# Youncy-Hu/MAGE

Measured on AMD Instinct MI355X. Metric: generated frames/sec (64x64, 16-frame clips), higher is better.
Workload: dtype bf16

## Files before the change

### mage_amd/config.py

```python
from __future__ import annotations

import contextlib
import dataclasses
import os
from typing import Iterator

__all__ = ["Config", "ENV", "get", "override", "lib_option", "lib_options", "lib_flag", "LIB_OPTIONS"]


@dataclasses.dataclass(frozen=True)
class Config:
    qk_fuse: bool = True
    mlp_fuse: bool = True
    ln_fold: bool = True
    stream_16bit: bool = True
    attn_split: bool = True
    frame_table: bool = True
    auto_graph: bool = True
    encode_split: bool = True
    decode_table: bool = True
    decode_split: bool = True
    decode_taps8: bool = True
    decode_resblock_fusion: bool = True
    decode_head_fusion: bool = True
    decode_phase_merge: bool = True
    decode_relu_fold: bool = True
    train_f32_branch: bool = False
    train_wgrad_transpose: bool = False
    train_emit: bool = True
    train_dual: bool = True
    train_taps: bool = True
    train_enc_split: bool = True


ENV = {
    "ln_fold": ("MAGE_NO_LN_FOLD", False),
    "qk_fuse": ("MAGE_NO_QK_FUSE", False),
    "mlp_fuse": ("MAGE_NO_MLP_FUSE", False),
    "stream_16bit": ("MAGE_STREAM_FP32", False),
    "attn_split": ("MAGE_ATTN_SPLIT_FP32", False),
    "frame_table": ("MAGE_NO_FRAME_TABLE", False),
    "auto_graph": ("MAGE_NO_AUTO_GRAPH", False),
    "encode_split": ("MAGE_ENCODE_FP32", False),
    "decode_table": ("MAGE_NO_DECODE_TABLE", False),
    "decode_split": ("MAGE_DECODE_FP32", False),
    "decode_taps8": ("MAGE_DECODE_NO_TAPS8", False),
    "decode_resblock_fusion": ("MAGE_DECODE_NO_RESBLOCK_FUSION", False),
    "decode_head_fusion": ("MAGE_DECODE_NO_HEAD_FUSION", False),
    "decode_phase_merge": ("MAGE_DECODE_NO_PHASE_MERGE", False),
    "decode_relu_fold": ("MAGE_DECODE_NO_RELU_FOLD", False),
    "train_f32_branch": ("MAGE_TRAIN_F32_BRANCH", True),
    "train_wgrad_transpose": ("MAGE_WGRAD_TRANSPOSE", True),
    "train_emit": ("MAGE_TRAIN_NO_EMIT", False),
    "train_dual": ("MAGE_TRAIN_NO_DUAL", False),
    "train_taps": ("MAGE_TRAIN_NO_TAPS", False),
    "train_enc_split": ("MAGE_TRAIN_ENC_FP32", False),
}

LIB_OPTIONS = ("gemm_no_4w", "gemm_no_4h", "gemm_4h_plain", "gemm4_train_forms", "gemm_no_8phase", "gemm_no_taps8", "gemm_no_narrow", "gemm_no_narrow_few", "gemm_no_small",
               "gemm_small_m", "gemm_stagger_groups", "gemm_stagger_percent", "gemm_stagger_forced",
               "gemm4_stagger_groups", "gemm4_stagger_percent", "attn_no_mfma", "attn_no_fewq", "vq_no_mfma", "conv_no_tile")


def _set(v) -> bool:
    return bool(v) and v != "0"


def _from_env() -> Config:
    kw = {}
    for field, (var, when_set) in ENV.items():
# ... 75 lines not shown
```

### mage_amd/csrc/gemm4.hip

```cpp
#include <cstdio>
#include <cstdlib>
#include <utility>

#include "gemm_shared.h"
#include "gemm4_regs.h"
#include "attn_mfma.h"

namespace {

struct Gemm4Args {
    const void* A;
    const void* W;
    void* Y;
    const float* bias;
    const float* ln_stats;
    const float* ln_colsum;
    const void* residual;
    float* ln_part;
    void* y2;
    int M, N, K, lda, ldw, ldy, ldr, ldy2, y_dtype, a_off, y_off;
    int ntiles_n, ntiles;
    int stagger_groups, stagger_sleeps;
    alignas(16) int attn_axis;
    float attn_scale;
// ... 23 lines not shown
#ifdef MAGE4_MFMA32
template <int B, bool ZERO, bool CLOB>
__device__ __forceinline__ void g4_mfma32(const u32x4& w, const u32x4& x) {
    if constexpr (ZERO && CLOB) asm volatile("v_mfma_f32_32x32x16_bf16 a[%c2:%c3], %0, %1, 0" ::"v"(w), "v"(x), "i"(16 * B), "i"(16 * B + 15) : G4_ALL_ACC);
    else if constexpr (ZERO) asm volatile("v_mfma_f32_32x32x16_bf16 a[%c2:%c3], %0, %1, 0" ::"v"(w), "v"(x), "i"(16 * B), "i"(16 * B + 15));
    else if constexpr (CLOB) asm volatile("v_mfma_f32_32x32x16_bf16 a[%c2:%c3], %0, %1, a[%c2:%c3]" ::"v"(w), "v"(x), "i"(16 * B), "i"(16 * B + 15) : G4_ALL_ACC);
    else asm volatile("v_mfma_f32_32x32x16_bf16 a[%c2:%c3], %0, %1, a[%c2:%c3]" ::"v"(w), "v"(x), "i"(16 * B), "i"(16 * B + 15));
}
#endif
typedef unsigned g4_u32x2 __attribute__((ext_vector_type(2)));
template <bool HF>
__device__ __forceinline__ f32x4 g4_epi_qk(const u32x4& k, const u32x4& q) {
    f32x4 d;
    if constexpr (HF) asm volatile("s_nop 1\n\tv_mfma_f32_16x16x32_f16 %0, %1, %2, 0\n\ts_nop 15" : "=&v"(d) : "v"(k), "v"(q));
    else asm volatile("s_nop 1\n\tv_mfma_f32_16x16x32_bf16 %0, %1, %2, 0\n\ts_nop 15" : "=&v"(d) : "v"(k), "v"(q));
    return d;
}
#define G4_EPI_PV(OP)                                                                                                                               \
    asm volatile("s_nop 1\n\t" OP " %0, %2, %4, 0\n\t" OP " %1, %3, %4, 0\n\t" OP " %0, %2, %5, %0\n\t" OP " %1, %3, %5, %1\n\ts_nop 15"           \
                 : "=&v"(o0), "=&v"(o1)                                                                                                             \
                 : "v"(__builtin_bit_cast(g4_u32x2, vt0)), "v"(__builtin_bit_cast(g4_u32x2, vt1)), "v"(__builtin_bit_cast(g4_u32x2, phi)),          \
                   "v"(__builtin_bit_cast(g4_u32x2, plo)))
template <bool HF>
__device__ __forceinline__ void g4_epi_pv(const ashort4& vt0, const ashort4& vt1, const ashort4& phi, const ashort4& plo, f32x4& o0, f32x4& o1) {
    if constexpr (HF) G4_EPI_PV("v_mfma_f32_16x16x16_f16");
    else G4_EPI_PV("v_mfma_f32_16x16x16_bf16");
}

template <bool SWAP, int I, bool ZERO, bool CLOB, bool HF>
__device__ __forceinline__ void g4_mm(const u32x4& w, const u32x4& x) {
    if constexpr (SWAP) g4_mfma<I, ZERO, CLOB, HF>(x, w);
    else g4_mfma<I, ZERO, CLOB, HF>(w, x);
}
template <int ACT, int EK, int LN, bool RB, bool HF, bool QF>
__device__ __forceinline__ void gemm4_body(const Gemm4Args& g) {
    static_assert(EK != EK_GENERAL, "lean epilogue kinds");
    static_assert(!QF || (LN == LN_CONSUME && ACT == MAGE_ACT_NONE), "fused attention: the LayerNorm-consuming in_proj");
    static_assert(!HF || (LN != LN_DUAL && LN != LN_GELUBWD), "f16 form: the generation path's epilogues");
    typedef std::conditional_t<HF, f16_t, unsigned short> H16;
    extern __shared__ __attribute__((aligned(16))) char smem[];
    g4_claim_accumulators();
    const int tid = threadIdx.x;
    const int lane = tid & 63;
    const int wave = __builtin_amdgcn_readfirstlane(tid >> 6);
    const int nwg8 = gridDim.x >> 3;
    const int xcd = blockIdx.x & 7, li = blockIdx.x >> 3;
    const int q8 = g.ntiles >> 3, r8 = g.ntiles & 7;
    const int chunk0 = xcd < r8 ? xcd * (q8 + 1) : r8 * (q8 + 1) + (xcd - r8) * q8;
    const int chunk1 = chunk0 + q8 + (xcd < r8 ? 1 : 0);
    const int nk = g.K >> 6;
    int c_tile = chunk0 + li;
    if (c_tile >= chunk1) return;
    const int last_tile = c_tile + ((chunk1 - 1 - c_tile) / nwg8) * nwg8;

    const int lr = lane >> 3, lp = lane & 7;
    unsigned voffA[8], voffW[8];
    [[maybe_unused]] auto frame_row = [&](int R) { return g.attn_axis == 1 ? ((R & 15) << 4) + (R >> 4) : R; };
#pragma unroll
    for (int u = 0; u < 8; ++u) {
        const int r = u * 8 + lr;
        const int ch = lp ^ ((r >> 1) & 7);
        voffA[u] = (unsigned)((QF ? frame_row(wave * 64 + r) : r) * g.lda * 2 + ch * 16 + 8192 - u * 1024);
        voffW[u] = (unsigned)(r * g.ldw * 2 + ch * 16 + 8192 - u * 1024);
    }
    auto a_base = [&](int tile) { return (const char*)g.A + ((long)((tile / g.ntiles_n) * 256 + (QF ? 0 : wave * 64)) + g.a_off) * g.lda * 2 - 4096; };
    auto w_base = [&](int tile) { return (const char*)g.W + (long)((tile % g.ntiles_n) * (QF ? 384 : 256) + wave * 64) * g.ldw * 2 - 4096; };
    [[maybe_unused]] auto w_base_v = [&](int tile) { return (const char*)g.W + (long)((tile % g.ntiles_n) * 384 + 256 + wave * 32) * g.ldw * 2 - 4096; };
    const char* a_src = a_base(c_tile);
    const char* w_src = w_base(c_tile);
    const char* a_next = a_src;
    const char* w_next = w_src;
    const unsigned lds0 = (unsigned)(uintptr_t)(__attribute__((address_space(3))) char*)smem + wave * 8192 + 4096;
    auto dma_m0 = [&](unsigned lds_group) __attribute__((always_inline)) {
        asm volatile("s_mov_b32 m0, %0\n\ts_nop 0" ::"s"(lds0 + lds_group) : "memory");
    };
    auto dma_m0w = [&](unsigned stage_off, bool half) __attribute__((always_inline)) { dma_m0(stage_off + G4_WOFF - (half ? wave * 4096 : 0)); };

    const int wm = wave >> 1, wn = wave & 1;
    const int l15 = lane & 15, grp = lane >> 4;
    const int rsw = (l15 >> 1) & 7;
    const int pc[2] = {((grp + 0) ^ rsw) * 16, ((grp + 4) ^ rsw) * 16};
    const int x_off = (wm * 128 + l15) * 128;
    const int w_off = G4_WOFF + (wn * 128 + l15) * 128;
    [[maybe_unused]] const int w_off_v = G4_WOFF + (wn * 64 + l15) * 128;
    u32x4 wf[2][8], xf[2][4];
    auto rd_w1 = [&](int buf, int stage, int t, int nt) __attribute__((always_inline)) {
        wf[buf][nt] = *(const u32x4*)(smem + stage * G4_STAGE + w_off + nt * 2048 + pc[t]);
    };
    [[maybe_unused]] auto rd_wv = [&](int buf, int stage, int t, int nt) __attribute__((always_inline)) {
        wf[buf][nt] = *(const u32x4*)(smem + stage * G4_STAGE + w_off_v + nt * 2048 + pc[t]);
    };
    auto rd_x1 = [&](int buf, int stage, int t, int mt) __attribute__((always_inline)) {
        xf[buf][mt & 3] = *(const u32x4*)(smem + stage * G4_STAGE + x_off + mt * 2048 + pc[t]);
    };

#ifdef MAGE4_MFMA32
    const int l31 = lane & 31, hi5 = lane >> 5;
    const int rsw32 = (l31 >> 1) & 7;
// ... 9 lines not shown
    if (g.stagger_groups > 1) {
        for (int w = (li % g.stagger_groups) * g.stagger_sleeps; w > 0; --w) __builtin_amdgcn_s_sleep(16);
    }
    dma_m0(0);
    g4_for<8>([&](auto u_) { g4_dma<decltype(u_)::value>(voffA[decltype(u_)::value], a_src); });
    dma_m0(G4_WOFF);
    g4_for<8>([&](auto u_) { g4_dma<decltype(u_)::value>(voffW[decltype(u_)::value], w_src); });
    a_src += 128;
    w_src += 128;
    dma_m0(G4_STAGE);
    g4_for<8>([&](auto u_) { g4_dma<decltype(u_)::value>(voffA[decltype(u_)::value], a_src); });
    dma_m0(G4_STAGE + G4_WOFF);
    g4_for<8>([&](auto u_) { g4_dma<decltype(u_)::value>(voffW[decltype(u_)::value], w_src); });
    a_src += 128;
    w_src += 128;
    __builtin_amdgcn_s_waitcnt(0x0F70);
    ring_barrier();
#ifdef MAGE4_MFMA32
#pragma unroll
    for (int b = 0; b < 4; ++b) { rd_w32(0, 0, 0, b); rd_x32(0, 0, 0, b); }
#else
#pragma unroll
    for (int nt = 0; nt < 8; ++nt) rd_w1(0, 0, 0, nt);
#pragma unroll
    for (int m = 0; m < 4; ++m) rd_x1(0, 0, 0, m);
#endif

    [[maybe_unused]] int it = 0;
    for (; c_tile < chunk1; c_tile += nwg8, ++it) {
        G4_STAMP(it, 0);
        const int tm = c_tile / g.ntiles_n, tn = c_tile - tm * g.ntiles_n;
        MAGE_DASSERT(c_tile >= 0 && c_tile < g.ntiles && tm * 256 < g.M && tn * (QF ? 384 : 256) < g.N);
        [[maybe_unused]] float ln_mean[8], ln_rstd[8];
        auto tile = [&](auto PH_) __attribute__((always_inline)) {
            constexpr int PH = decltype(PH_)::value;
            constexpr bool HALF = PH == 2, KEEP = PH == 1;
            constexpr int NW = HALF ? 4 : 8;
            const int m0 = ((MAGE4_ABL & 32) ? (int)blockIdx.x : tm) * 256 + wm * 128;
            const int n0 = QF ? tn * 384 + (HALF ? 256 + wn * 64 : wn * 128) : ((MAGE4_ABL & 32) ? 0 : tn) * 256 + wn * 128;
            [[maybe_unused]] const int ny0 = HALF ? tn * 128 + wn * 64 : n0;
            if constexpr (KEEP) {
                a_next = a_base(c_tile);
                w_next = w_base_v(c_tile);
            } else {
                const int nt_tile = c_tile + nwg8 > last_tile ? last_tile : c_tile + nwg8;
                a_next = a_base(nt_tile);
                w_next = w_base(nt_tile);
            }
            auto rd_w = [&](int buf, int stage, int t, int nt) __attribute__((always_inline)) {
                if constexpr (HALF) rd_wv(buf, stage, t, nt);
                else rd_w1(buf, stage, t, nt);
            };
            f32x4 biasm[2][4];
            [[maybe_unused]] f32x4 lns[2][4];
            [[maybe_unused]] f32x4 pl[4][2];
            [[maybe_unused]] int ql15 = l15, qgrp = grp;
            if constexpr (QF) asm volatile("" : "+v"(ql15), "+v"(qgrp));
            auto slab = [&](auto S_, auto FIRST_, auto LAST_, int j) __attribute__((always_inline)) {
                constexpr int S = decltype(S_)::value;
                constexpr bool FIRST = decltype(FIRST_)::value, LAST = decltype(LAST_)::value;
                constexpr int ACC0 = HALF ? 32 : 0;
                constexpr bool WH_ = LAST ? KEEP : HALF;
                constexpr int WU = WH_ ? 4 : 8;
                g4_for<4 * NW>([&](auto i_) {
                    constexpr int i = decltype(i_)::value, m = i / NW, nt = i % NW;
                    g4_mm<PH == 2, ACC0 + ((nt >> 2) * 8 + m) * 4 + (nt & 3), FIRST, i == 0, HF>(wf[0][nt], xf[0][m]);
                    __builtin_amdgcn_sched_barrier(0);
                    if constexpr (!(MAGE4_ABL & 4) && i < 4) {
                        rd_x1(1, S, 0, 4 + i);
                        __builtin_amdgcn_sched_barrier(0);
                    }
                    if constexpr (!(MAGE4_ABL & 2) && !FIRST && i == 4) {
                        dma_m0w((S ^ 1) * G4_STAGE, WH_);
                        __builtin_amdgcn_sched_barrier(0);
                    }
// ... 9 lines not shown
                        }
                    }
                });
                if constexpr (!(MAGE4_ABL & 2) && !FIRST && !HALF && WU == 8) {
                    g4_dma<7>(voffW[7], w_src);
                    __builtin_amdgcn_sched_barrier(0);
                }
                if constexpr (!(MAGE4_ABL & 8) && !FIRST) w_src = (j == nk - 2) ? w_next : w_src + 128;
                g4_for<4 * NW>([&](auto i_) {
                    constexpr int i = decltype(i_)::value, m = i / NW, nt = i % NW;
                    g4_mm<PH == 2, ACC0 + ((nt >> 2) * 8 + 4 + m) * 4 + (nt & 3), FIRST, i == 0, HF>(wf[0][nt], xf[1][m]);
                    __builtin_amdgcn_sched_barrier(0);
                    if constexpr (!(MAGE4_ABL & 4) && i < 4 + NW) {
                        if constexpr (i < 4) rd_x1(0, S, 1, i);
                        else rd_w(1, S, 1, i - 4);
                        __builtin_amdgcn_sched_barrier(0);
                    }
                });
                if constexpr (LAST) {
#pragma unroll
                    for (int b = 0; b < 4; ++b) {
                        if constexpr (PH == 2) {
                            biasm[0][0][b] = g.bias[n0 + b * 16 + l15];
                            lns[0][0][b] = g.ln_colsum[n0 + b * 16 + l15];
                            continue;
                        }
                        const int n = n0 + b * 16 + grp * 4;
                        biasm[0][b] = *(const f32x4*)(g.bias + n);
                        if constexpr (LN == LN_CONSUME) lns[0][b] = *(const f32x4*)(g.ln_colsum + n);
                    }
                    if constexpr (LN == LN_CONSUME && !HALF) {
#pragma unroll
                        for (int a = 0; a < 8; ++a) {
                            const long row = QF ? (long)tm * 256 + frame_row(wm * 128 + a * 16 + ql15) : (long)(m0 + a * 16 + l15);
                            const float2 st = *(const float2*)(g.ln_stats + 2 * row);
                            ln_mean[a] = st.x;
                            ln_rstd[a] = st.y;
                        }
                    }
                    __builtin_amdgcn_sched_barrier(0);
                }
                g4_for<4 * NW>([&](auto i_) {
                    constexpr int i = decltype(i_)::value, m = i / NW, nt = i % NW;
                    g4_mm<PH == 2, ACC0 + ((nt >> 2) * 8 + m) * 4 + (nt & 3), false, i == 0, HF>(wf[1][nt], xf[0][m]);
                    __builtin_amdgcn_sched_barrier(0);
                    if constexpr (!(MAGE4_ABL & 4) && i < 4) {
                        rd_x1(1, S, 1, 4 + i);
                        __builtin_amdgcn_sched_barrier(0);
                    }
                });
                if constexpr (MAGE4_ABL & 16) __builtin_amdgcn_s_waitcnt(0xC07F);
                else if constexpr (FIRST && QF) __builtin_amdgcn_s_waitcnt(PH == 1 ? 0x007C : 0x0070);
                else if constexpr (FIRST) __builtin_amdgcn_s_waitcnt(LN == LN_CONSUME ? 0x8074 : 0x8070);
                else __builtin_amdgcn_s_waitcnt(0x0070);
                ring_barrier();
                __builtin_amdgcn_sched_barrier(0);
                g4_for<4 * NW>([&](auto i_) {
                    constexpr int i = decltype(i_)::value, m = i / NW, nt = i % NW;
                    g4_mm<PH == 2, ACC0 + ((nt >> 2) * 8 + 4 + m) * 4 + (nt & 3), false, i == 0, HF>(wf[1][nt], xf[1][m]);
                    __builtin_amdgcn_sched_barrier(0);
                    if constexpr (!(MAGE4_ABL & 4) && i < 4 + NW && !LAST) {
                        if constexpr (i < 4) rd_x1(0, S ^ 1, 0, i);
                        else rd_w(0, S ^ 1, 0, i - 4);
                        __builtin_amdgcn_sched_barrier(0);
                    }
                    if constexpr (!(MAGE4_ABL & 2) && !LAST && !HALF) {
                        if constexpr (i == 2) dma_m0(S * G4_STAGE);
// ... 99 lines not shown
                    biasm[1][0][b] = g.bias[n0 + 64 + b * 16 + l15];
                    lns[1][0][b] = g.ln_colsum[n0 + 64 + b * 16 + l15];
                    continue;
                }
                const int n = n0 + 64 + b * 16 + grp * 4;
                biasm[1][b] = *(const f32x4*)(g.bias + n);
                if constexpr (LN == LN_CONSUME) lns[1][b] = *(const f32x4*)(g.ln_colsum + n);
            }
            if constexpr (QF) {
                g4_for<(HALF ? 2 : 4)>([&](auto c_) {
                    constexpr int c = decltype(c_)::value, h = HALF ? 0 : c >> 1, mh = c & 1, ha = HALF ? 1 : h;
                    __builtin_amdgcn_sched_barrier(0);
                    f32x4 t[4][4];
                    g4_for<16>([&](auto q_) {
                        constexpr int q = decltype(q_)::value;
                        t[q >> 2][q & 3] = g4_acc_read<(ha * 8 + mh * 4 + (q >> 2)) * 4 + (q & 3), q == 0>();
                    });
                    if constexpr (PH == 1) {
#pragma unroll
                        for (int mt = 0; mt < 4; ++mt) {
                            uint2 pk[4];
#pragma unroll
                            for (int nt = 0; nt < 4; ++nt) {
                                const f32x4 v = (t[mt][nt] - lns[h][nt] * ln_mean[mh * 4 + mt]) * ln_rstd[mh * 4 + mt] + biasm[h][nt];
                                pk[nt] = uint2{pack16x2<H16>(v[0], v[1]), pack16x2<H16>(v[2], v[3])};
                            }
                            f32x4 st = g4_epi_qk<HF>(u32x4{pk[2].x, pk[2].y, pk[3].x, pk[3].y}, u32x4{pk[0].x, pk[0].y, pk[1].x, pk[1].y});
                            f32x4 p;
                            {
#pragma clang fp contract(off)
                                float mx = -INFINITY;
#pragma unroll
                                for (int e = 0; e < 4; ++e) {
                                    st[e] = st[e] * g.attn_scale;
                                    mx = fmaxf(mx, st[e]);
                                }
                                mx = fmaxf(mx, __shfl_xor(mx, 16));
                                mx = fmaxf(mx, __shfl_xor(mx, 32));
#pragma unroll
                                for (int e = 0; e < 4; ++e) p[e] = expf(st[e] - mx);
                            }
                            pl[mt][0] = p;
                        }
                        g4_for<4>([&](auto mt_) { g4_acc_write<c * 4 + decltype(mt_)::value>(pl[decltype(mt_)::value][0]); });
                    } else {
                        const long shift = (long)(tm * 256 / g.out_w) * (g.y_img_stride - g.out_w) + g.y_off;
                        const int srow = (qgrp * 16 + ql15) >> 3, scc = ql15 & 7;
                        H16* op = (H16*)g.Y + ny0 + h * 64 + scc * 8;
                        const int wchunk = (qgrp & 1) * 2 + (qgrp >> 1);
                        g4_for<8>([&](auto q_) {
                            constexpr int q = decltype(q_)::value, hd = q >> 2, mt = q & 3;
                            pl[mt][hd] = g4_acc_read<(hd * 2 + mh) * 4 + mt>();
                        });
#pragma unroll
                        for (int mt = 0; mt < 4; ++mt) {
                            f32x4 mean4, rstd4;
#pragma unroll
                            for (int e = 0; e < 4; ++e) {
                                mean4[e] = __shfl(ln_mean[mh * 4 + mt], 4 * grp + e);
                                rstd4[e] = __shfl(ln_rstd[mh * 4 + mt], 4 * grp + e);
                            }
#pragma unroll
                            for (int hd = 0; hd < 2; ++hd) {
                                const f32x4 p = pl[mt][hd];
                                float den = 0.f;
                                ashort4 phi, plo;
#pragma unroll
                                for (int e = 0; e < 4; ++e) {
                                    den += p[e];
                                    short ph, pw;
                                    attn_p_split<H16>(p[e], ph, pw);
                                    phi[e] = ph;
                                    plo[e] = pw;
                                }
                                den += __shfl_xor(den, 16);
                                den += __shfl_xor(den, 32);
                                f32x4 o[2];
                                ashort4 vt[2];
#pragma unroll
                                for (int b = 0; b < 2; ++b) {
                                    const int nt = hd * 2 + b;
                                    const f32x4 v = (t[mt][nt] - mean4 * lns[h][0][nt]) * rstd4 + biasm[h][0][nt];
                                    vt[b] = __builtin_bit_cast(ashort4, uint2{pack16x2<H16>(v[0], v[1]), pack16x2<H16>(v[2], v[3])});
                                }
                                g4_epi_pv<HF>(vt[0], vt[1], phi, plo, o[0], o[1]);
                                const float inv = 1.0f / den;
                                f32x4 v0, v1;
#pragma unroll
                                for (int e = 0; e < 4; ++e) {
                                    const auto sw = __builtin_amdgcn_permlane16_swap(__float_as_uint(o[0][e]), __float_as_uint(o[1][e]), false, false);
                                    v0[e] = __uint_as_float(sw[0]) * inv;
                                    v1[e] = __uint_as_float(sw[1]) * inv;
                                }
                                *(u32x4*)(win + ql15 * 128 + (((hd * 4 + wchunk) ^ ((ql15 >> 1) & 7)) << 4)) =
                                    u32x4{pack16x2<H16>(v0[0], v0[1]), pack16x2<H16>(v0[2], v0[3]), pack16x2<H16>(v1[0], v1[1]), pack16x2<H16>(v1[2], v1[3])};
                            }
#pragma unroll
                            for (int i = 0; i < 2; ++i) {
                                const int r = srow + 8 * i;
                                const long yrow = (long)tm * 256 + frame_row(wm * 128 + mh * 64 + mt * 16 + r) + shift;
                                *(u32x4*)(op + yrow * g.ldy) = *(const u32x4*)(win + r * 128 + ((scc ^ ((r >> 1) & 7)) << 4));
                            }
                        }
                    }
                });
            } else {
            mage_gemm_desc e = {};
            e.M = 0x7fffffff;
            e.N = LN == LN_PRODUCE ? g.N : 0x7fffffff;
            e.K = g.K;
            e.Y = g.Y;
            e.ldy = g.ldy;
            e.y_dtype = g.y_dtype;
            e.out_h = 1;
            e.out_w = 0x7fffffff;
            e.y_mul_x = 1;
            e.y_off = g.y_off;
            e.y2 = g.y2;
            e.ldy2 = g.ldy2;
            e.ln_part = g.ln_part;
            g4_for<4>([&](auto c_) {
                constexpr int c = decltype(c_)::value, h = c >> 1, mh = c & 1;
                __builtin_amdgcn_sched_barrier(0);
                f32x4 t[4][4];
                g4_for<16>([&](auto q_) {
                    constexpr int q = decltype(q_)::value;
                    t[q >> 2][q & 3] = g4_acc_read<(h * 8 + mh * 4 + (q >> 2)) * 4 + (q & 3), q == 0>();
                });
                [[maybe_unused]] LnConsume lnc;
                if constexpr (LN == LN_CONSUME) {
#pragma unroll
                    for (int a = 0; a < 4; ++a) {
                        lnc.mean[a] = ln_mean[mh * 4 + a];
// ... 18 lines not shown
#pragma unroll
                for (int nt = 0; nt < 4; ++nt) rd_wv(0, 0, 0, nt);
#pragma unroll
                for (int m = 0; m < 4; ++m) rd_x1(0, 0, 0, m);
            } else if (c_tile + nwg8 < chunk1) {
#ifdef MAGE4_MFMA32
#pragma unroll
                for (int b = 0; b < 4; ++b) { rd_w32(0, 0, 0, b); rd_x32(0, 0, 0, b); }
#else
#pragma unroll
                for (int nt = 0; nt < 8; ++nt) rd_w1(0, 0, 0, nt);
#pragma unroll
                for (int m = 0; m < 4; ++m) rd_x1(0, 0, 0, m);
#endif
            }
        };
        if constexpr (QF) {
            tile(std::integral_constant<int, 1>{});
            tile(std::integral_constant<int, 2>{});
        } else {
            tile(std::integral_constant<int, 0>{});
        }
    }
}

template <int ACT, int EK, int LN, bool RB, bool HF = false>
__global__ __launch_bounds__(256) void gemm4_kernel(const Gemm4Args g) {
    gemm4_body<ACT, EK, LN, RB, HF, false>(g);
}
template <bool HF>
__global__ __launch_bounds__(256) void gemm4_attn_kernel(const Gemm4Args g) {
    gemm4_body<MAGE_ACT_NONE, EK_BIAS, LN_CONSUME, false, HF, true>(g);
}

template <int ACT, int EK, int LN, bool RB, bool HF = false, bool QF = false>
int launch4(const mage_gemm_desc* d, hipStream_t s, int n_cu, int attn_axis = 0, float attn_scale = 0.f) {
    Gemm4Args a;
    a.attn_axis = attn_axis;
    a.attn_scale = attn_scale;
    a.out_w = d->out_w;
    a.y_img_stride = d->y_img_stride;
    a.A = d->A;
    a.W = d->W;
    a.Y = d->Y;
    a.bias = d->bias ? d->bias : (const float*)mage_zero_page();
    a.ln_stats = d->ln_stats;
    a.ln_colsum = d->ln_colsum;
    a.residual = d->residual;
    a.ln_part = d->ln_part;
    a.y2 = d->y2;
    a.M = d->M;
    a.N = d->N;
    a.K = d->K;
    a.lda = d->lda;
    a.ldw = d->ldw ? d->ldw : d->K;
    a.ldy = d->ldy;
    a.ldr = d->ldr;
    a.ldy2 = d->ldy2;
    a.y_dtype = d->y_dtype;
    a.a_off = d->a_off;
    a.y_off = d->y_off;
    a.ntiles_n = d->N / (QF ? 384 : 256);
    a.ntiles = (d->M / 256) * a.ntiles_n;
    const int st_groups = mage_options().gemm4_stagger_groups, st_percent = mage_options().gemm4_stagger_percent;
    a.stagger_groups = 0;
    a.stagger_sleeps = 0;
    const int grid = a.ntiles >= n_cu ? n_cu : ((a.ntiles + 7) & ~7);
    if (st_groups > 1 && a.ntiles / grid >= 6) {
        const long period = (long)(d->K / 64) * 3100 + 9000;
        a.stagger_groups = st_groups;
        a.stagger_sleeps = (int)(period * st_percent / 100 / st_groups / 1024);
    }
    int r;
    if constexpr (QF) r = mage_gemm_launch<gemm4_attn_kernel<HF>>(grid, 256, G4_LDS, s, a);
    else r = mage_gemm_launch<gemm4_kernel<ACT, EK, LN, RB, HF>>(grid, 256, G4_LDS, s, a);
    return r < 0 ? r : 1;
}

}

namespace {

struct Tn4Args {
    const unsigned short* A;
    const unsigned short* B;
    float* P;
    float* DB;
    long lda, ldb, T, tps;
    int N, K, n_split, ntk;
};
typedef short g4_tr4 __attribute__((ext_vector_type(4)));
__device__ __forceinline__ g4_tr4 g4_lds_tr(const char* p) { return __builtin_amdgcn_ds_read_tr16_b64_v4i16((__attribute__((address_space(3))) g4_tr4*)p); }

template <bool DB>
__global__ __launch_bounds__(256) void gemm_tn4_kernel(const Tn4Args g) {
    constexpr int PART = 32768, STAGE = 2 * PART;
    extern __shared__ __attribute__((aligned(16))) char smem[];
    g4_claim_accumulators();
    const int lane = threadIdx.x & 63;
    const int wave = __builtin_amdgcn_readfirstlane(threadIdx.x >> 6);
    const int tile = blockIdx.x / g.n_split, s = blockIdx.x - tile * g.n_split;
    const int tm = tile / g.ntk, tk = tile - tm * g.ntk;
    const long t_begin = (long)s * g.tps;
    const long t_end = t_begin + g.tps < g.T ? t_begin + g.tps : g.T;
    const int nslab = (int)((t_end - t_begin) >> 6);
    const int rr = lane >> 3, pc = lane & 7;
    unsigned voffA[8], voffB[8];
// ... 192 lines not shown
    if ((dual || gbwd) && (d->y_dtype != MAGE_BF16 || d->ldy2 % 8 || (((uintptr_t)d->y2) & 15))) return 0;
    if (!dual && !gbwd && d->act != MAGE_ACT_NONE && d->act != MAGE_ACT_QUICKGELU) return 0;
    if (d->y_dtype != MAGE_F32 && d->y_dtype != d->dtype) return 0;
    if (hf && (dual || gbwd)) return 0;
    if (d->ldy % 8 || d->lda % 8 || (((uintptr_t)d->bias | (uintptr_t)d->ln_colsum) & 15) || (((uintptr_t)d->ln_stats) & 7)) return 0;
    const int n_cu = mage_gemm_cu_count();
    const long ntiles = (long)(d->M / 256) * (d->N / 256);
    const bool few_tiles = ntiles < 4L * n_cu;
    const int ldw = d->ldw ? d->ldw : d->K;
    if (((long)d->M + d->a_off) * d->lda * 2 + 16384 >= (1L << 32) || (long)d->N * ldw * 2 + 16384 >= (1L << 32)) return 0;
    if (!dual && !gbwd)
        if (const int r = mage_gemm4h_try(d, s, n_cu)) return r;
    if (few_tiles) return 0;
    if (dual) return launch4<MAGE_ACT_QUICKGELU, EK_BIAS, LN_DUAL, false>(d, s, n_cu);
    if (gbwd) return launch4<MAGE_ACT_NONE, EK_BIAS, LN_GELUBWD, false>(d, s, n_cu);
    if (hf) {
        if (d->ln_stats) {
            if (d->act == MAGE_ACT_NONE) return launch4<MAGE_ACT_NONE, EK_BIAS, LN_CONSUME, false, true>(d, s, n_cu);
            return launch4<MAGE_ACT_QUICKGELU, EK_BIAS, LN_CONSUME, false, true>(d, s, n_cu);
        }
        if (d->act == MAGE_ACT_NONE) return launch4<MAGE_ACT_NONE, EK_BIAS, LN_NONE, false, true>(d, s, n_cu);
        return launch4<MAGE_ACT_QUICKGELU, EK_BIAS, LN_NONE, false, true>(d, s, n_cu);
    }
    if (d->ln_stats) {
        if (d->act == MAGE_ACT_NONE) return launch4<MAGE_ACT_NONE, EK_BIAS, LN_CONSUME, false>(d, s, n_cu);
        return launch4<MAGE_ACT_QUICKGELU, EK_BIAS, LN_CONSUME, false>(d, s, n_cu);
    }
    if (d->act == MAGE_ACT_NONE) return launch4<MAGE_ACT_NONE, EK_BIAS, LN_NONE, false>(d, s, n_cu);
    return launch4<MAGE_ACT_QUICKGELU, EK_BIAS, LN_NONE, false>(d, s, n_cu);
}

extern "C" int mage_gemm_attn_fused_qkv(const mage_gemm_desc* d, int32_t axis, float scale, void* stream) {
    MAGE_CHECK_ARG(d != nullptr, "mage_gemm_attn_fused_qkv: null descriptor");
    MAGE_CHECK_ARG(axis == 1 || axis == 2, "mage_gemm_attn_fused_qkv: axis %d (1 = H, 2 = W of 16 x 16 frames)", (int)axis);
    MAGE_CHECK_ARG(d->dtype == MAGE_BF16 || d->dtype == MAGE_F16, "mage_gemm_attn_fused_qkv: bf16 or f16 operands");
    MAGE_CHECK_ARG(d->A && d->W && d->Y && d->bias && d->ln_stats && d->ln_colsum, "mage_gemm_attn_fused_qkv: A, W, Y, bias, ln_stats, ln_colsum must be given");
    MAGE_CHECK_ARG(d->M > 0 && d->M % 256 == 0 && d->N > 0 && d->N % 384 == 0 && d->K % 128 == 0 && d->K >= 256 && d->K <= 1024,
                   "mage_gemm_attn_fused_qkv: M=%d a multiple of 256 (whole 16 x 16 frames), N=%d = 3C a multiple of 384 (groups of 4 heads of width 32), K=%d a "
                   "multiple of 128 in [256, 1024]", d->M, d->N, d->K);
    MAGE_CHECK_ARG(d->taps_h * d->taps_w == 1 && d->stride == 1 && !d->dy0 && !d->dx0 && d->in_h == 1 && d->out_h == 1 && d->in_w == d->out_w && !d->a_half &&
                       d->y_mul_x == 1 && (d->out_w >= d->M || (d->out_w % 256 == 0 && d->a_img_stride == d->out_w)) && d->a_off % 256 == 0 && d->a_off >= 0,
                   "mage_gemm_attn_fused_qkv: plain rows in (a_off a multiple of 256), output rows regrouped whole frames at a time");
    MAGE_CHECK_ARG(!d->scale && !d->shift && !d->rowadd && !d->residual && !d->post_relu && !d->res_half && !d->y2 && !d->ln_part && !d->head_w && !d->a_relu &&
                       d->n_split <= 1 && d->act == MAGE_ACT_NONE,
                   "mage_gemm_attn_fused_qkv: the LayerNorm-consuming bias epilogue only");
    MAGE_CHECK_ARG(d->y_dtype == d->dtype && d->ldy % 8 == 0 && d->ldy >= d->N / 3 && (((uintptr_t)d->Y) & 15) == 0 && d->y_off >= 0,
                   "mage_gemm_attn_fused_qkv: 16-bit output rows of the operands' type, ldy a multiple of 8 and >= C, Y 16-byte aligned");
    const int ldw = d->ldw ? d->ldw : d->K;
    MAGE_CHECK_ARG(ldw == d->K && d->lda % 8 == 0 && d->lda >= d->K, "mage_gemm_attn_fused_qkv: W packed [N][K], lda a multiple of 8");
    MAGE_CHECK_ARG((((uintptr_t)d->A | (uintptr_t)d->W | (uintptr_t)d->bias | (uintptr_t)d->ln_colsum) & 15) == 0 && (((uintptr_t)d->ln_stats) & 7) == 0,
                   "mage_gemm_attn_fused_qkv: operands must be 16-byte aligned");
    MAGE_CHECK_ARG(((long)d->M + d->a_off) * d->lda * 2 + 16384 < (1L << 32) && (long)d->N * ldw * 2 + 16384 < (1L << 32),
                   "mage_gemm_attn_fused_qkv: operands beyond the kernel's 32-bit lane offsets");
    hipStream_t s = (hipStream_t)stream;
    const int n_cu = mage_gemm_cu_count();
    const int r = d->dtype == MAGE_F16 ? launch4<MAGE_ACT_NONE, EK_BIAS, LN_CONSUME, false, true, true>(d, s, n_cu, axis, scale)
                                       : launch4<MAGE_ACT_NONE, EK_BIAS, LN_CONSUME, false, false, true>(d, s, n_cu, axis, scale);
    return r < 0 ? r : MAGE_OK;
}

extern "C" int mage_gemm_attn_fused_qkv_kernel_name(const mage_gemm_desc* d, int32_t axis, char* buf, int32_t len) {
    MAGE_CHECK_ARG(buf != nullptr && len > 0, "mage_gemm_attn_fused_qkv_kernel_name: no buffer");
    const void* kernel = nullptr;
    mage_gemm_plan = &kernel;
    const int r = mage_gemm_attn_fused_qkv(d, axis, 1.f, nullptr);
    mage_gemm_plan = nullptr;
    if (r != MAGE_OK) return r;
    return mage_kernel_symbol_name(kernel, buf, len, "mage_gemm_attn_fused_qkv_kernel_name");
}

int mage_gemm_tn4_try(const void* dY, int64_t lda, const void* X, int64_t ldb, int64_t T, int32_t N, int32_t K, int32_t n_split, int64_t tps,
                      float* partials, float* db_partials, hipStream_t stream) {
    if (mage_options().gemm_no_4w) return 0;
    if (T % 64 || tps % 64 || tps < 128 || (T - (int64_t)(n_split - 1) * tps) < 128) return 0;
    if (lda * 2 * 64 + 16384 >= (1L << 31) || ldb * 2 * 64 + 16384 >= (1L << 31)) return 0;
    const int dev = mage_device_index();
    if (dev < 0) return 0;
    static bool attr[MAGE_MAX_DEVICES] = {false};
    if (!attr[dev]) {
        (void)hipFuncSetAttribute((const void*)gemm_tn4_kernel<false>, hipFuncAttributeMaxDynamicSharedMemorySize, 128 * 1024);
        (void)hipFuncSetAttribute((const void*)gemm_tn4_kernel<true>, hipFuncAttributeMaxDynamicSharedMemorySize, 128 * 1024);
        attr[dev] = true;
    }
    Tn4Args a;
    a.A = (const unsigned short*)dY;
    a.B = (const unsigned short*)X;
    a.P = partials;
    a.DB = db_partials;
    a.lda = lda;
    a.ldb = ldb;
// ... 13 lines not shown
```

### mage_amd/modules/mage_model.py

```python
from __future__ import annotations

import contextlib
import ctypes
import gc
import math
from collections import OrderedDict
from math import exp
from typing import Dict, Optional, Tuple

import torch
from torch import nn

from .. import config, ops
from ..utils.util import default, instantiate_from_config, zero_module
from .vqvae_model import VectorQuantizedVAE, _Derived, _conv_w, _no_torch_forward, weights_frozen

__all__ = ["QuickGELU", "AxialAttentionBlock", "TransformerBlock", "MAEncoder", "TransformerTextEncoder", "BasicBlock",
           "ADAIN2D", "FlatAxialDecoder", "PIDControl", "MAGE"]

F32 = torch.float32
BF16 = torch.bfloat16
F16 = torch.float16
HALF_TYPES = (BF16, F16)

# ... 392 lines not shown

    def _fold(self, dt, B: int, hw: int) -> bool:
        return (dt in HALF_TYPES and (B * hw) % 256 == 0 and self.model_channels % 256 == 0 and config.get().ln_fold)

    def _stream_bf16(self) -> bool:
        return getattr(self, "stream_bf16", True) and config.get().stream_16bit

    def _ln_linear(self, d, p, lin, xn, xb, ln, y, *, M, N, sk=0, **kw):
        Cc, name = self.model_channels, f"{p}.{lin}"
        if ln is None:
            return _linear(xn, d, name, y, self.compute_dtype, M=M, N=N, K=Cc, sk=sk, **kw)
        lnw, lns = self._ln_fold_w(d, p, lin, xb.dtype)
        return ops.gemm(xb, lnw, y, M=M, N=N, K=Cc, lda=Cc, ldy=N, bias=d[name + ".lnc"], ln_colsum=lns, **ln, **kw)

    @staticmethod
    def _ln_fold_w(d, p, lin, dt):
        if dt == BF16:
            return d[f"{p}.{lin}.lnw"], d[f"{p}.{lin}.lns"]
        kw_, ks_ = f"{p}.{lin}.lnw.f16", f"{p}.{lin}.lns.f16"
        if kw_ not in d:
            ln = "ln_1" if lin == "in_proj" else "ln_2"
            wq = (d[f"{p}.{lin}.f32"] * d[f"{p}.{ln}.w"][None, :]).to(F16)
            d[kw_], d[ks_] = wq, wq.float().sum(dim=1).contiguous()
        return d[kw_], d[ks_]

    def _qkv_fuse(self, xb, M: int, hh: int, ww: int, stats_rows: bool, cache) -> bool:
        Cc = self.model_channels
        if not (stats_rows and cache is None and hh == 16 and ww == 16 and self.use_cids and config.get().qk_fuse):
            return False
        if Cc % 256 or not 256 <= Cc <= 1024 or M % 256 or (M + 8) * Cc * 2 >= 2 ** 32:
            return False
        return (M // 256) * (Cc // 128) >= getattr(self, "qkv_fuse_tiles", 8) * torch.cuda.get_device_properties(xb.device).multi_processor_count

    def _mlp_fuse(self, xb, M: int, stats_rows: bool, sb: bool) -> bool:
        if not (stats_rows and sb and self.use_cids and self.model_channels == 512 and config.get().mlp_fuse):
            return False
        if M % 128 or M * 512 >= 2 ** 31:
            return False
        return M // 128 >= getattr(self, "mlp_fuse_tiles", 8) * torch.cuda.get_device_properties(xb.device).multi_processor_count

    def _qkv_fuse_w(self, d, p, dt):
        sfx = ".f16" if dt == F16 else ""
        if f"{p}.in_proj.qkv.w{sfx}" not in d:
            lnw, lns = self._ln_fold_w(d, p, "in_proj", dt)
            self._qkv_fuse_pack(d, p, lnw, lns, sfx)
        q = f"{p}.in_proj.qkv."
        return dict(w=d[q + "w" + sfx], s=d[q + "s" + sfx], c=d[q + "c"])

    def _qkv_fuse_pack(self, d, p, lnw, lns, sfx: str) -> None:
        idx = ops.qkv_pack_rows(self.model_channels, lnw.device)
        d[f"{p}.in_proj.qkv.w{sfx}"], d[f"{p}.in_proj.qkv.s{sfx}"] = lnw[idx].contiguous(), lns[idx].contiguous()
        d[f"{p}.in_proj.qkv.c"] = d[f"{p}.in_proj.lnc"][idx].contiguous()

    def _stats_inline(self, xb, M: int) -> bool:
        Cc = self.model_channels
        return all(ops.gemm_is_small(xb, M, n, Cc) for n in (Cc, 2 * Cc, 3 * Cc, 4 * Cc))

    @torch.no_grad()
    def _run(self, motion: torch.Tensor, imgs: torch.Tensor, *, B: int, hh: int, ww: int) -> torch.Tensor:
        L = self.frames_length
        return self._pass(motion, imgs, B=B, hh=hh, ww=ww, p0=0, P=L, nf=L - 1, cache=None)

    def _inc_begin(self, B: int, hh: int, ww: int) -> dict:
        return {"B": B, "hh": hh, "ww": ww, "kv": {}, "p": 0}

    @torch.no_grad()
# ... 47 lines not shown
    def _pass(self, motion, imgs, *, B: int, hh: int, ww: int, p0: int, P: int, nf: int, cache: Optional[dict],
              nh: Optional[int] = None) -> torch.Tensor:
        d = self._derived.get(self._build)
        dt, Cc, L = self.compute_dtype, self.model_channels, self.frames_length
        dev = (imgs.tokens if isinstance(imgs, FrameTokens) else imgs).device
        hw = hh * ww
        M = B * P * hw
        sk = self._sk()
        qs = bool(sk) and self._attn_split()
        cw = 2 * Cc if qs else Cc
        fold = not sk and self._fold(dt, B, hw)
        sb = fold and self._stream_bf16()
        xb = part = stats = None
        if fold:
            xb = torch.empty(M, Cc, device=dev, dtype=dt)
            part = torch.empty(Cc // 64, M, 2, device=dev, dtype=F32)
            stats = torch.empty(M, 2, device=dev, dtype=F32)
        inl = fold and self._stats_inline(xb, M)
        ln = None if not fold else dict(ln_part=part, ln_eps=1e-5) if inl else dict(ln_stats=stats)
        ln0 = dict(ln_stats=stats) if sb else None
        x = xb if sb else torch.empty(M, Cc, device=dev, dtype=F32)
        res = dict(residual=x, ldr=Cc)
        if fold:
            res["ln_part"] = part
            if not sb:
                res.update(y2=xb, ldy2=Cc)
        self._embed(d, x, motion, imgs, B=B, hw=hw, P=P, nf=nf, tp=d["tpos"][p0:])
        if sb:
            ops.row_stats(xb, 1e-5, stats)

        def rows(n, split=bool(sk), m=M):
            return ops.split_empty(m, n, sk, dev) if split else torch.empty(m, n, device=dev, dtype=dt)

        xn, qkv, ao = rows(Cc), rows(3 * Cc, qs), rows(Cc)
        geo = [self._axial_geo(a, B, hh, ww, P, p0, cached=cache is not None, q_cached=cache is not None and not sk) for a in range(3)]
        fuse = not sk and self._qkv_fuse(xb, M, hh, ww, fold and not inl, cache)
        mfuse = not sk and self._mlp_fuse(xb, M, fold and not inl, sb)
        hdn = None if mfuse else rows(4 * Cc)
        for i in range(self.layers):
            p = f"b{i}"
            ln1 = ln if i else ln0
            if ln1 is None:
                ops.layernorm(x, d[p + ".ln_1.w"], d[p + ".ln_1.b"], xn, 1e-5, split_kind=sk)
            if fuse and i % 3:
                f = self._qkv_fuse_w(d, p, dt)
                ops.gemm_attn_fused_qkv(xb, f["w"], ao, axis=i % 3, M=M, C_=Cc, K=Cc, lda=Cc, ldy=Cc, bias=f["c"], ln_stats=stats, ln_colsum=f["s"])
            elif i % 3 == 0 and cache is not None and not sk:
                if p0 == 0:
                    cache[i] = rows(3 * Cc, m=B * L * hw)
                kv = cache[i]
                self._ln_linear(d, p, "in_proj", xn, xb, ln1, kv, M=M, N=3 * Cc, out_w=P * hw, y_img_stride=L * hw, y_off=p0 * hw)
                q, k, v = kv[p0 * hw:], kv[:, cw:], kv[:, 2 * cw:]
            elif i % 3 == 0 and cache is not None:
                if p0 == 0:
                    cache[i] = rows(2 * Cc, qs, B * L * hw)
                k = cache[i]
                q, v = qkv.view(-1)[:M * cw].view(M, cw), k[:, cw:]
                _linear(xn, d, p + ".in_proj", q, dt, M=M, N=Cc, K=Cc, sk=sk, lo=0, hi=Cc)
                _linear(xn, d, p + ".in_proj", k, dt, M=M, N=2 * Cc, K=Cc, sk=sk, lo=Cc, hi=3 * Cc, out_w=P * hw, y_img_stride=L * hw,
                        y_off=p0 * hw)
            else:
                q, k, v = qkv, qkv[:, cw:], qkv[:, 2 * cw:]
                self._ln_linear(d, p, "in_proj", xn, xb, ln1, qkv, M=M, N=3 * Cc, sk=sk)
            if not (fuse and i % 3):
                ops.attention(q, k, v, ao, ldq=q.stride(0), ldk=k.stride(0), ldv=v.stride(0), ldo=ao.stride(0), out_split=sk,
                              split_kind=sk if qs else 0, **geo[i % 3])
            _linear(ao, d, p + ".out_proj", x, dt, M=M, N=Cc, K=Cc, sk=sk, **res)
            if fold and not inl:
                ops.ln_stats(part, Cc, 1e-5, stats)
            if ln is None:
                ops.layernorm(x, d[p + ".ln_2.w"], d[p + ".ln_2.b"], xn, 1e-5, split_kind=sk)
            if mfuse:
                lnw, lns = self._ln_fold_w(d, p, "c_fc", dt)
                last = i == self.layers - 1
                ops.mlp_fused(xb, xn if last else xb, M=M, C_=Cc, w1=lnw, c1=d[p + ".c_fc.lnc"], s1=lns, ln_stats=stats,
                              w2=_wdt(d, p + ".c_proj", dt), b2=d[p + ".c_proj.b"], ln_part=None if last else part)
                if last:
                    xa = xn
                else:
                    ops.ln_stats(part, Cc, 1e-5, stats)
                continue
            self._ln_linear(d, p, "c_fc", xn, xb, ln, hdn, M=M, N=4 * Cc, sk=sk, act=ops.ACT_QUICKGELU)
            if i < self.layers - 1:
                _linear(hdn, d, p + ".c_proj", x, dt, M=M, N=Cc, K=4 * Cc, sk=sk, **res)
                if fold and not inl:
                    ops.ln_stats(part, Cc, 1e-5, stats)
            else:
                if self.use_cids and (sk or dt != F32):
                    xa = xn
                else:
                    xa = torch.empty(M, Cc, device=dev, dtype=F32) if sb else x
                _linear(hdn, d, p + ".c_proj", xa, dt, M=M, N=Cc, K=4 * Cc, sk=sk, residual=x, ldr=Cc)
        return self._head(d, xa, B=B, hw=hw, P=P, nf=nf if nh is None else nh)

    def _split_on(self) -> bool:
        return bool(self.split_kind) and self.compute_dtype == F32 and self.model_channels % 64 == 0

# ... 1563 lines not shown
```

Measured before the change: 6530.

## Fuse temporal-axis attention into the LayerNorm-consuming QKV GEMM kernel

Extends the fused in_proj+attention GEMM kernel to the temporal axis (axis 0). It adds a row map that gathers the 16 frame slots of each spatial position from a clip, plus a causal mask in the softmax. The model now routes temporal layers through this fused path when there is no cache and a full 16-frame clip, and skips allocating the qkv buffer when every layer is fused. This removes the qkv write/read round trip and a separate attention launch for the temporal layers. The cost is strided A-row gathers across frames, which may coalesce worse than contiguous tiles.

New measurement: 6662, median of 6. 2.0% higher.

```diff
diff --git a/mage_amd/config.py b/mage_amd/config.py
--- a/mage_amd/config.py
+++ b/mage_amd/config.py
@@ -11,6 +11,7 @@
 @dataclasses.dataclass(frozen=True)
 class Config:
     qk_fuse: bool = True
+    tqkv_fuse: bool = True
     mlp_fuse: bool = True
     ln_fold: bool = True
     stream_16bit: bool = True
@@ -36,6 +37,7 @@
 ENV = {
     "ln_fold": ("MAGE_NO_LN_FOLD", False),
     "qk_fuse": ("MAGE_NO_QK_FUSE", False),
+    "tqkv_fuse": ("MAGE_NO_TQKV_FUSE", False),
     "mlp_fuse": ("MAGE_NO_MLP_FUSE", False),
     "stream_16bit": ("MAGE_STREAM_FP32", False),
     "attn_split": ("MAGE_ATTN_SPLIT_FP32", False),
diff --git a/mage_amd/csrc/gemm4.hip b/mage_amd/csrc/gemm4.hip
--- a/mage_amd/csrc/gemm4.hip
+++ b/mage_amd/csrc/gemm4.hip
@@ -79,9 +79,10 @@
     if constexpr (SWAP) g4_mfma<I, ZERO, CLOB, HF>(x, w);
     else g4_mfma<I, ZERO, CLOB, HF>(w, x);
 }
-template <int ACT, int EK, int LN, bool RB, bool HF, bool QF>
+template <int ACT, int EK, int LN, bool RB, bool HF, bool QF, bool TX = false>
 __device__ __forceinline__ void gemm4_body(const Gemm4Args& g) {
     static_assert(EK != EK_GENERAL, "lean epilogue kinds");
+    static_assert(!TX || QF, "the temporal row map belongs to the fused attention entry");
     static_assert(!QF || (LN == LN_CONSUME && ACT == MAGE_ACT_NONE), "fused attention: the LayerNorm-consuming in_proj");
     static_assert(!HF || (LN != LN_DUAL && LN != LN_GELUBWD), "f16 form: the generation path's epilogues");
     typedef std::conditional_t<HF, f16_t, unsigned short> H16;
@@ -102,15 +103,26 @@
 
     const int lr = lane >> 3, lp = lane & 7;
     unsigned voffA[8], voffW[8];
-    [[maybe_unused]] auto frame_row = [&](int R) { return g.attn_axis == 1 ? ((R & 15) << 4) + (R >> 4) : R; };
+    [[maybe_unused]] auto frame_row = [&](int R) {
+        if constexpr (TX) return (R & 15) * g.out_w + (R >> 4);
+        else return g.attn_axis == 1 ? ((R & 15) << 4) + (R >> 4) : R;
+    };
+    [[maybe_unused]] auto tile_row0 = [&](int tm_) {
+        const int clip = tm_ / g.y_img_stride;
+        return (long)clip * 16 * g.out_w + (tm_ - clip * g.y_img_stride) * 16;
+    };
 #pragma unroll
     for (int u = 0; u < 8; ++u) {
         const int r = u * 8 + lr;
         const int ch = lp ^ ((r >> 1) & 7);
-        voffA[u] = (unsigned)((QF ? frame_row(wave * 64 + r) : r) * g.lda * 2 + ch * 16 + 8192 - u * 1024);
+        if constexpr (TX) voffA[u] = (unsigned)frame_row(wave * 64 + r) * (unsigned)(g.lda * 2) + (unsigned)(ch * 16 + 8192 - u * 1024);
+        else voffA[u] = (unsigned)((QF ? frame_row(wave * 64 + r) : r) * g.lda * 2 + ch * 16 + 8192 - u * 1024);
         voffW[u] = (unsigned)(r * g.ldw * 2 + ch * 16 + 8192 - u * 1024);
     }
-    auto a_base = [&](int tile) { return (const char*)g.A + ((long)((tile / g.ntiles_n) * 256 + (QF ? 0 : wave * 64)) + g.a_off) * g.lda * 2 - 4096; };
+    auto a_base = [&](int tile) {
+        if constexpr (TX) return (const char*)g.A + (tile_row0(tile / g.ntiles_n) + g.a_off) * g.lda * 2 - 4096;
+        else return (const char*)g.A + ((long)((tile / g.ntiles_n) * 256 + (QF ? 0 : wave * 64)) + g.a_off) * g.lda * 2 - 4096;
+    };
     auto w_base = [&](int tile) { return (const char*)g.W + (long)((tile % g.ntiles_n) * (QF ? 384 : 256) + wave * 64) * g.ldw * 2 - 4096; };
     [[maybe_unused]] auto w_base_v = [&](int tile) { return (const char*)g.W + (long)((tile % g.ntiles_n) * 384 + 256 + wave * 32) * g.ldw * 2 - 4096; };
     const char* a_src = a_base(c_tile);
@@ -186,6 +198,8 @@
         const int tm = c_tile / g.ntiles_n, tn = c_tile - tm * g.ntiles_n;
         MAGE_DASSERT(c_tile >= 0 && c_tile < g.ntiles && tm * 256 < g.M && tn * (QF ? 384 : 256) < g.N);
         [[maybe_unused]] float ln_mean[8], ln_rstd[8];
+        [[maybe_unused]] long row0 = 0;
+        if constexpr (TX) row0 = tile_row0(tm);
         auto tile = [&](auto PH_) __attribute__((always_inline)) {
             constexpr int PH = decltype(PH_)::value;
             constexpr bool HALF = PH == 2, KEEP = PH == 1;
@@ -194,7 +208,8 @@
             const int n0 = QF ? tn * 384 + (HALF ? 256 + wn * 64 : wn * 128) : ((MAGE4_ABL & 32) ? 0 : tn) * 256 + wn * 128;
             [[maybe_unused]] const int ny0 = HALF ? tn * 128 + wn * 64 : n0;
             if constexpr (KEEP) {
-                a_next = a_base(c_tile);
+                if constexpr (TX) a_next = (const char*)g.A + (row0 + g.a_off) * g.lda * 2 - 4096;
+                else a_next = a_base(c_tile);
                 w_next = w_base_v(c_tile);
             } else {
                 const int nt_tile = c_tile + nwg8 > last_tile ? last_tile : c_tile + nwg8;
@@ -270,7 +285,9 @@
                     if constexpr (LN == LN_CONSUME && !HALF) {
 #pragma unroll
                         for (int a = 0; a < 8; ++a) {
-                            const long row = QF ? (long)tm * 256 + frame_row(wm * 128 + a * 16 + ql15) : (long)(m0 + a * 16 + l15);
+                            long row;
+                            if constexpr (TX) row = row0 + frame_row(wm * 128 + a * 16 + ql15);
+                            else row = QF ? (long)tm * 256 + frame_row(wm * 128 + a * 16 + ql15) : (long)(m0 + a * 16 + l15);
                             const float2 st = *(const float2*)(g.ln_stats + 2 * row);
                             ln_mean[a] = st.x;
                             ln_rstd[a] = st.y;
@@ -436,19 +453,25 @@
                                 float mx = -INFINITY;
 #pragma unroll
                                 for (int e = 0; e < 4; ++e) {
-                                    st[e] = st[e] * g.attn_scale;
+                                    if constexpr (TX) st[e] = (4 * qgrp + e <= ql15) ? st[e] * g.attn_scale : -INFINITY;
+                                    else st[e] = st[e] * g.attn_scale;
                                     mx = fmaxf(mx, st[e]);
                                 }
                                 mx = fmaxf(mx, __shfl_xor(mx, 16));
                                 mx = fmaxf(mx, __shfl_xor(mx, 32));
 #pragma unroll
-                                for (int e = 0; e < 4; ++e) p[e] = expf(st[e] - mx);
+                                for (int e = 0; e < 4; ++e) {
+                                    if constexpr (TX) p[e] = (4 * qgrp + e <= ql15) ? expf(st[e] - mx) : 0.f;
+                                    else p[e] = expf(st[e] - mx);
+                                }
                             }
                             pl[mt][0] = p;
                         }
                         g4_for<4>([&](auto mt_) { g4_acc_write<c * 4 + decltype(mt_)::value>(pl[decltype(mt_)::value][0]); });
                     } else {
-                        const long shift = (long)(tm * 256 / g.out_w) * (g.y_img_stride - g.out_w) + g.y_off;
+                        long shift;
+                        if constexpr (TX) shift = g.y_off;
+                        else shift = (long)(tm * 256 / g.out_w) * (g.y_img_stride - g.out_w) + g.y_off;
                         const int srow = (qgrp * 16 + ql15) >> 3, scc = ql15 & 7;
                         H16* op = (H16*)g.Y + ny0 + h * 64 + scc * 8;
                         const int wchunk = (qgrp & 1) * 2 + (qgrp >> 1);
@@ -502,7 +525,9 @@
 #pragma unroll
                             for (int i = 0; i < 2; ++i) {
                                 const int r = srow + 8 * i;
-                                const long yrow = (long)tm * 256 + frame_row(wm * 128 + mh * 64 + mt * 16 + r) + shift;
+                                long yrow;
+                                if constexpr (TX) yrow = row0 + frame_row(wm * 128 + mh * 64 + mt * 16 + r) + shift;
+                                else yrow = (long)tm * 256 + frame_row(wm * 128 + mh * 64 + mt * 16 + r) + shift;
                                 *(u32x4*)(op + yrow * g.ldy) = *(const u32x4*)(win + r * 128 + ((scc ^ ((r >> 1) & 7)) << 4));
                             }
                         }
@@ -587,14 +612,19 @@
 __global__ __launch_bounds__(256) void gemm4_attn_kernel(const Gemm4Args g) {
     gemm4_body<MAGE_ACT_NONE, EK_BIAS, LN_CONSUME, false, HF, true>(g);
 }
-
-template <int ACT, int EK, int LN, bool RB, bool HF = false, bool QF = false>
+template <bool HF>
+__global__ __launch_bounds__(256) void gemm4_tattn_kernel(const Gemm4Args g) {
+    gemm4_body<MAGE_ACT_NONE, EK_BIAS, LN_CONSUME, false, HF, true, true>(g);
+}
+
+template <int ACT, int EK, int LN, bool RB, bool HF = false, bool QF = false, bool TX = false>
 int launch4(const mage_gemm_desc* d, hipStream_t s, int n_cu, int attn_axis = 0, float attn_scale = 0.f) {
     Gemm4Args a;
     a.attn_axis = attn_axis;
     a.attn_scale = attn_scale;
     a.out_w = d->out_w;
     a.y_img_stride = d->y_img_stride;
+    if constexpr (TX) a.y_img_stride = d->out_w / 16;
     a.A = d->A;
     a.W = d->W;
     a.Y = d->Y;
@@ -627,7 +657,8 @@
         a.stagger_sleeps = (int)(period * st_percent / 100 / st_groups / 1024);
     }
     int r;
-    if constexpr (QF) r = mage_gemm_launch<gemm4_attn_kernel<HF>>(grid, 256, G4_LDS, s, a);
+    if constexpr (TX) r = mage_gemm_launch<gemm4_tattn_kernel<HF>>(grid, 256, G4_LDS, s, a);
+    else if constexpr (QF) r = mage_gemm_launch<gemm4_attn_kernel<HF>>(grid, 256, G4_LDS, s, a);
     else r = mage_gemm_launch<gemm4_kernel<ACT, EK, LN, RB, HF>>(grid, 256, G4_LDS, s, a);
     return r < 0 ? r : 1;
 }
@@ -886,14 +917,26 @@
 
 extern "C" int mage_gemm_attn_fused_qkv(const mage_gemm_desc* d, int32_t axis, float scale, void* stream) {
     MAGE_CHECK_ARG(d != nullptr, "mage_gemm_attn_fused_qkv: null descriptor");
-    MAGE_CHECK_ARG(axis == 1 || axis == 2, "mage_gemm_attn_fused_qkv: axis %d (1 = H, 2 = W of 16 x 16 frames)", (int)axis);
+    MAGE_CHECK_ARG(axis >= 0 && axis <= 2, "mage_gemm_attn_fused_qkv: axis %d (0 = T of clips of 16 slots, 1 = H, 2 = W of 16 x 16 frames)", (int)axis);
+    if (axis == 0) {
+        const long hw = d->out_w;
+        MAGE_CHECK_ARG(hw >= 16 && hw % 16 == 0 && d->M > 0 && d->M % (16 * hw) == 0,
+                       "mage_gemm_attn_fused_qkv: axis 0: out_w=%d (the rows of one slot) a multiple of 16, M=%d whole clips of 16 slots", d->out_w, d->M);
+        MAGE_CHECK_ARG(d->y_img_stride == d->out_w && d->a_img_stride == d->out_w,
+                       "mage_gemm_attn_fused_qkv: axis 0: rows are not regrouped (y_img_stride=%d, a_img_stride=%d must equal out_w=%d)", d->y_img_stride,
+                       d->a_img_stride, d->out_w);
+        MAGE_CHECK_ARG(d->a_off % (16 * hw) == 0 && d->y_off % (16 * hw) == 0, "mage_gemm_attn_fused_qkv: axis 0: a_off=%d and y_off=%d must be whole clips", d->a_off,
+                       d->y_off);
+        MAGE_CHECK_ARG(d->lda > 0 && (15 * hw + 16) * d->lda * 2 + 16384 < (1L << 32),
+                       "mage_gemm_attn_fused_qkv: axis 0: a clip's rows beyond the kernel's 32-bit lane offsets");
+    }
     MAGE_CHECK_ARG(d->dtype == MAGE_BF16 || d->dtype == MAGE_F16, "mage_gemm_attn_fused_qkv: bf16 or f16 operands");
     MAGE_CHECK_ARG(d->A && d->W && d->Y && d->bias && d->ln_stats && d->ln_colsum, "mage_gemm_attn_fused_qkv: A, W, Y, bias, ln_stats, ln_colsum must be given");
     MAGE_CHECK_ARG(d->M > 0 && d->M % 256 == 0 && d->N > 0 && d->N % 384 == 0 && d->K % 128 == 0 && d->K >= 256 && d->K <= 1024,
                    "mage_gemm_attn_fused_qkv: M=%d a multiple of 256 (whole 16 x 16 frames), N=%d = 3C a multiple of 384 (groups of 4 heads of width 32), K=%d a "
                    "multiple of 128 in [256, 1024]", d->M, d->N, d->K);
     MAGE_CHECK_ARG(d->taps_h * d->taps_w == 1 && d->stride == 1 && !d->dy0 && !d->dx0 && d->in_h == 1 && d->out_h == 1 && d->in_w == d->out_w && !d->a_half &&
-                       d->y_mul_x == 1 && (d->out_w >= d->M || (d->out_w % 256 == 0 && d->a_img_stride == d->out_w)) && d->a_off % 256 == 0 && d->a_off >= 0,
+                       d->y_mul_x == 1 && (axis == 0 || d->out_w >= d->M || (d->out_w % 256 == 0 && d->a_img_stride == d->out_w)) && d->a_off % 256 == 0 && d->a_off >= 0,
                    "mage_gemm_attn_fused_qkv: plain rows in (a_off a multiple of 256), output rows regrouped whole frames at a time");
     MAGE_CHECK_ARG(!d->scale && !d->shift && !d->rowadd && !d->residual && !d->post_relu && !d->res_half && !d->y2 && !d->ln_part && !d->head_w && !d->a_relu &&
                        d->n_split <= 1 && d->act == MAGE_ACT_NONE,
@@ -908,8 +951,13 @@
                    "mage_gemm_attn_fused_qkv: operands beyond the kernel's 32-bit lane offsets");
     hipStream_t s = (hipStream_t)stream;
     const int n_cu = mage_gemm_cu_count();
-    const int r = d->dtype == MAGE_F16 ? launch4<MAGE_ACT_NONE, EK_BIAS, LN_CONSUME, false, true, true>(d, s, n_cu, axis, scale)
-                                       : launch4<MAGE_ACT_NONE, EK_BIAS, LN_CONSUME, false, false, true>(d, s, n_cu, axis, scale);
+    int r;
+    if (axis == 0)
+        r = d->dtype == MAGE_F16 ? launch4<MAGE_ACT_NONE, EK_BIAS, LN_CONSUME, false, true, true, true>(d, s, n_cu, axis, scale)
+                                 : launch4<MAGE_ACT_NONE, EK_BIAS, LN_CONSUME, false, false, true, true>(d, s, n_cu, axis, scale);
+    else
+        r = d->dtype == MAGE_F16 ? launch4<MAGE_ACT_NONE, EK_BIAS, LN_CONSUME, false, true, true>(d, s, n_cu, axis, scale)
+                                 : launch4<MAGE_ACT_NONE, EK_BIAS, LN_CONSUME, false, false, true>(d, s, n_cu, axis, scale);
     return r < 0 ? r : MAGE_OK;
 }
 
diff --git a/mage_amd/modules/mage_model.py b/mage_amd/modules/mage_model.py
--- a/mage_amd/modules/mage_model.py
+++ b/mage_amd/modules/mage_model.py
@@ -448,6 +448,14 @@
             return False
         return (M // 256) * (Cc // 128) >= getattr(self, "qkv_fuse_tiles", 8) * torch.cuda.get_device_properties(xb.device).multi_processor_count
 
+    def _tqkv_fuse(self, xb, M: int, hw: int, P: int, p0: int, stats_rows: bool, cache) -> bool:
+        Cc, cfg = self.model_channels, config.get()
+        if not (stats_rows and cache is None and P == 16 and p0 == 0 and hw % 16 == 0 and self.use_cids and cfg.qk_fuse and cfg.tqkv_fuse):
+            return False
+        if Cc % 256 or not 256 <= Cc <= 1024 or M % (16 * hw) or (M + 8) * Cc * 2 >= 2 ** 32 or (15 * hw + 16) * Cc * 2 + 16384 >= 2 ** 32:
+            return False
+        return (M // 256) * (Cc // 128) >= getattr(self, "qkv_fuse_tiles", 8) * torch.cuda.get_device_properties(xb.device).multi_processor_count
+
     def _mlp_fuse(self, xb, M: int, stats_rows: bool, sb: bool) -> bool:
         if not (stats_rows and sb and self.use_cids and self.model_channels == 512 and config.get().mlp_fuse):
             return False
@@ -561,9 +569,12 @@
         def rows(n, split=bool(sk), m=M):
             return ops.split_empty(m, n, sk, dev) if split else torch.empty(m, n, device=dev, dtype=dt)
 
-        xn, qkv, ao = rows(Cc), rows(3 * Cc, qs), rows(Cc)
         geo = [self._axial_geo(a, B, hh, ww, P, p0, cached=cache is not None, q_cached=cache is not None and not sk) for a in range(3)]
         fuse = not sk and self._qkv_fuse(xb, M, hh, ww, fold and not inl, cache)
+        tfuse = not sk and self._tqkv_fuse(xb, M, hw, P, p0, fold and not inl, cache)
+        fused = [(fuse if i % 3 else tfuse and (i > 0 or ln0 is not None)) for i in range(self.layers)]
+        xn, ao = rows(Cc), rows(Cc)
+        qkv = None if all(fused) else rows(3 * Cc, qs)
         mfuse = not sk and self._mlp_fuse(xb, M, fold and not inl, sb)
         hdn = None if mfuse else rows(4 * Cc)
         for i in range(self.layers):
@@ -571,9 +582,10 @@
             ln1 = ln if i else ln0
             if ln1 is None:
                 ops.layernorm(x, d[p + ".ln_1.w"], d[p + ".ln_1.b"], xn, 1e-5, split_kind=sk)
-            if fuse and i % 3:
+            if fused[i]:
                 f = self._qkv_fuse_w(d, p, dt)
-                ops.gemm_attn_fused_qkv(xb, f["w"], ao, axis=i % 3, M=M, C_=Cc, K=Cc, lda=Cc, ldy=Cc, bias=f["c"], ln_stats=stats, ln_colsum=f["s"])
+                ops.gemm_attn_fused_qkv(xb, f["w"], ao, axis=i % 3, M=M, C_=Cc, K=Cc, lda=Cc, ldy=Cc, bias=f["c"], ln_stats=stats, ln_colsum=f["s"],
+                                        out_w=None if i % 3 else hw)
             elif i % 3 == 0 and cache is not None and not sk:
                 if p0 == 0:
                     cache[i] = rows(3 * Cc, m=B * L * hw)
@@ -591,7 +603,7 @@
             else:
                 q, k, v = qkv, qkv[:, cw:], qkv[:, 2 * cw:]
                 self._ln_linear(d, p, "in_proj", xn, xb, ln1, qkv, M=M, N=3 * Cc, sk=sk)
-            if not (fuse and i % 3):
+            if not fused[i]:
                 ops.attention(q, k, v, ao, ldq=q.stride(0), ldk=k.stride(0), ldv=v.stride(0), ldo=ao.stride(0), out_split=sk,
                               split_kind=sk if qs else 0, **geo[i % 3])
             _linear(ao, d, p + ".out_proj", x, dt, M=M, N=Cc, K=Cc, sk=sk, **res)
```
